# NethermindEth/cairo_zstd

Measured on AMD Instinct MI355X. Metric: decompressed MB/s (whole node), 128 KiB-block batch, higher is better.
Workload: dtype u8

## Files before the change

### cairo_zstd_amd/csrc/czstd_chain.hip

```cpp
#include "czstd_dict.h"

#ifndef CZC_SLOTS
#define CZC_SLOTS 10
#endif
#define CZC_LPS 4
static_assert(CZC_SLOTS * CZC_LPS <= 64, "quads of one wave");
#define CZC_MAXSYM 64
#define CZC_RING 512u
#define CZC_STEPS 32u
static_assert(((CZC_STEPS * 58u + 7u) / 8u + 12u) + 12u <= 256u + 12u, "a top-up adds at most 256 bytes: one must be enough for the next group");
#define CZC_NEED ((CZC_STEPS * 58u + 7u) / 8u + 12u)
#define CZC_MAP_WORDS CZ_CHAIN_MAP_WORDS

#define CZC_E16(nb, base, xb) ((uint16_t)(((((1u << (9u - (nb))) | ((base) >> (nb))) << 6) | (xb))))
#define CZC_E16_IDLE 0x8000u

struct CzChainSlot {
    uint16_t t_ll[512], t_ml[512], t_of[256];
    union {
        struct {
            __attribute__((aligned(16))) uint8_t stage[256];
            int16_t probs[3][CZC_MAXSYM];
            uint16_t counters_ml[CZC_MAXSYM];
        };
// ... 6 lines not shown
struct CzChainShared { CzChainSlot slot[CZC_SLOTS]; uint32_t llml[96]; uint16_t idle[2]; };

__device__ static inline __attribute__((always_inline)) int czc_fse_build_wave(uint16_t* table, const int16_t* probs, uint32_t nprobs, uint32_t log,
                                                                   uint8_t* symof, uint16_t* counters, const uint32_t* llml, uint32_t kind, cz_gptr map) {
    const uint32_t size = 1u << log, mask = size - 1, lim = kind == 0 ? 36u : (kind == 1 ? 32u : 53u);
    const uint32_t lane = (uint32_t)LANE;
    const unsigned long long lt = (1ull << lane) - 1ull;
    const int32_t p = lane < nprobs ? (int32_t)probs[lane] : 0;
    if (__ballot(p != 0 && lane >= lim)) return 1;
    const unsigned long long lowm = __ballot(p == -1);
    const uint32_t neg = size - (uint32_t)__popcll(lowm);
    if (p == -1) table[size - 1u - (uint32_t)__popcll(lowm & lt)] = (uint16_t)lane;
    counters[lane] = 0;
    const uint32_t cnt = p > 0 ? (uint32_t)p : 0u;
    const uint32_t cum = cz_wave_incl_scan(cnt) - cnt;
    for (uint32_t i = 4u * lane; i < size; i += 256u) *(uint32_t*)(symof + i) = 0u;
    cz_wave_sync();
    if (cnt && cum < size) symof[cum] = (uint8_t)lane;
    cz_wave_sync();
    {
        const uint32_t per = size >= 64u ? size >> 6 : 1u, b0 = lane * per;
        const int act = b0 < size;
        uint32_t run = 0, vals[8];
#pragma unroll
        for (uint32_t j = 0; j < 8; j++) { if (act && j < per) { const uint32_t v = symof[b0 + j]; run = v > run ? v : run; } vals[j] = run; }
        uint32_t inc = act ? run : 0u;
#define CZC_MAX_STEP(CTRL, RM) do { const uint32_t o_ = cz_dpp<CTRL, RM>(0u, inc); inc = o_ > inc ? o_ : inc; } while (0)
        CZC_MAX_STEP(CZ_DPP_SHR1, 0xF); CZC_MAX_STEP(CZ_DPP_SHR2, 0xF); CZC_MAX_STEP(CZ_DPP_SHR4, 0xF); CZC_MAX_STEP(CZ_DPP_SHR8, 0xF);
        CZC_MAX_STEP(CZ_DPP_BCAST15, 0xA); CZC_MAX_STEP(CZ_DPP_BCAST31, 0xC);
#undef CZC_MAX_STEP
        const uint32_t exc = cz_dpp<CZ_DPP_WAVE_SHR1, 0xF>(0u, inc);
#pragma unroll
        for (uint32_t j = 0; j < 8; j++) if (act && j < per) symof[b0 + j] = (uint8_t)(vals[j] > exc ? vals[j] : exc);
    }
    cz_wave_sync();
    {
        const uint32_t step = (size >> 1) + (size >> 3) + 3u;
        uint32_t running = 0;
        for (uint32_t j0 = 0; j0 < size; j0 += 64u) {
            const uint32_t j = j0 + lane, pos = (j * step) & mask;
            const int valid = j < size && pos < neg;
            const unsigned long long vm = __ballot(valid);
            if (valid) table[pos] = symof[running + (uint32_t)__popcll(vm & lt)];
            running += (uint32_t)__popcll(vm);
        }
    }
    cz_wave_sync();
    for (uint32_t i0 = 0; i0 < size; i0 += 64u) {
        const uint32_t i = i0 + lane;
        const int in = i < size, cell = in && i < neg;
        const uint32_t s = in ? (uint32_t)table[i] : 0u;
        unsigned long long same = __ballot(cell);
#pragma unroll
        for (uint32_t b = 0; b < 6; b++) { const int bit = (int)((s >> b) & 1u); const unsigned long long m = __ballot(bit); same &= bit ? m : ~m; }
        const uint32_t n = cell ? (uint32_t)probs[s] : 1u;
        const uint32_t k = (cell ? (uint32_t)counters[s] : 0u) + (uint32_t)__popcll(same & lt);
        cz_wave_sync();
        if (cell && (same >> lane) == 1ull) counters[s] = (uint16_t)(k + 1u);
        const uint32_t xb = kind == 1 ? s : (llml[(kind == 2 ? 40u : 0u) + s] >> 24);
        uint32_t nb = log, bl = 0;
        if (cell) {
            const uint32_t m = 1u << (cz_hbs(n) - 1), slices = (m == n) ? n : m * 2;
            const uint32_t dbl = slices - n, single = n - dbl, width = size >> (cz_hbs(slices) - 1);
            nb = cz_hbs(width) - 1;
            if (k < dbl) { bl = single * width + k * width * 2; nb += 1; }
            else bl = (k - dbl) * width;
        }
        if (in) { table[i] = CZC_E16(nb, bl, xb); if (map) map[i] = (uint8_t)s; }
        cz_wave_sync();
    }
    return 0;
}

__device__ static inline uint4 czc_load16(uintptr_t a, uintptr_t S, uintptr_t E) {
    uint4 v;
    if (a >= S && a + 16 <= E) { __builtin_memcpy(&v, (CZ_GLOBAL const void*)a, 16); return v; }
    if (a + 16 <= S || a >= E) { v.x = v.y = v.z = v.w = 0; return v; }
    uint32_t w[4] = {0, 0, 0, 0};
    for (uint32_t b = 0; b < 16; b++) { const uintptr_t q = a + b; if (q >= S && q < E) w[b >> 2] |= (uint32_t)(*(cz_gcptr)q) << (8 * (b & 3)); }
    v.x = w[0]; v.y = w[1]; v.z = w[2]; v.w = w[3];
    return v;
}
#define CZC_PF (16 / CZC_LPS)
struct CzcPre { uint4 v[CZC_PF]; };
__device__ static inline void czc_prefetch(CzcPre& pre, int has_slot, intptr_t lo, uintptr_t Sk, uintptr_t Ek) {
    const uint32_t j = (uint32_t)LANE & 3u;
#pragma unroll
    for (uint32_t r = 0; r < CZC_PF; r++) {
        const uint32_t c = j + r * CZC_LPS;
        if (has_slot) pre.v[r] = czc_load16((uintptr_t)lo - 16u * (c + 1), Sk, Ek);
    }
}
__device__ static inline void czc_commit(CzChainSlot& sk, int has_slot, intptr_t old_lo, intptr_t new_lo, const CzcPre& pre) {
    const uint32_t j = (uint32_t)LANE & 3u;
    const uint32_t cnt = has_slot ? (uint32_t)(old_lo - new_lo) >> 4 : 0u;
#pragma unroll
    for (uint32_t r = 0; r < CZC_PF; r++) {
        const uint32_t c = j + r * CZC_LPS;
        if (c < cnt) {
            const uint32_t slot = (uint32_t)(((uintptr_t)old_lo - 16u * (c + 1)) & (CZC_RING - 1));
            *(uint4*)&sk.ring[slot] = pre.v[r];
            if (slot == CZC_RING - 16) { *(uint32_t*)&sk.mirror[4] = pre.v[r].y; *(uint32_t*)&sk.mirror[8] = pre.v[r].z; *(uint32_t*)&sk.mirror[12] = pre.v[r].w; }
        }
    }
}
__device__ static inline uint64_t czc_window(const CzChainSlot& sl, int32_t u) {
    const uint32_t ba = ((uint32_t)u >> 3) & (CZC_RING - 4), ph = (uint32_t)u & 31;
    const uint32_t w2 = *(const uint32_t*)(sl.ring + ba), w1 = *(const uint32_t*)(sl.ring + ba - 4), w0 = *(const uint32_t*)(sl.ring + ba - 8);
    const uint64_t hi = (((uint64_t)w2 << 32) | w1), lo = (((uint64_t)w1 << 32) | w0);
    const uint32_t h = ph ? (uint32_t)(hi >> ph) : w1, l = ph ? (uint32_t)(lo >> ph) : w0;
    return ((uint64_t)h << 32) | l;
}

struct CzcLane {
    uint32_t E;
    uint32_t S;
    int32_t  u;
    uint32_t ph;
    uint32_t w0, w1, w2;
    uint32_t slow;
};
struct CzcRole {
    const uint16_t* tb;
    const uint8_t* ringm8;
    uint32_t m1, m2;
    uint32_t sh;
    uint32_t lane0;
    uint32_t sbits;
};
#define CZC_QP(a, b, c, d) ((a) | ((b) << 2) | ((c) << 4) | ((d) << 6))
template <int CTRL> __device__ static inline uint32_t czc_qp(uint32_t v) { return (uint32_t)__builtin_amdgcn_update_dpp(0, (int)v, CTRL, 0xF, 0xF, true); }

__device__ static inline void czc_ring_words(CzcLane& c, const CzcRole& ro) {
    const uint8_t* ba = ro.ringm8 + (__builtin_amdgcn_ubfe((uint32_t)c.u, 5, 7) << 2);
    c.w0 = *(const uint32_t*)ba; c.w1 = *(const uint32_t*)(ba + 4); c.w2 = *(const uint32_t*)(ba + 8);
    c.ph = (uint32_t)c.u & 31u;
}
__device__ static inline uint32_t czc_bits32(const CzcRole& ro, uint32_t v) {
    const uint8_t* ba = ro.ringm8 + (__builtin_amdgcn_ubfe(v, 5, 7) << 2);
    return __builtin_amdgcn_alignbit(*(const uint32_t*)(ba + 8), *(const uint32_t*)(ba + 4), v & 31u);
}
#define CZC_WIDE_STEPS 16u
static_assert((CZC_WIDE_STEPS * 89u + 7u) / 8u + 12u <= CZC_NEED && CZC_STEPS % CZC_WIDE_STEPS == 0, "a redone asm group is whole wide groups, each within the staged bytes");
__device__ static inline void czc_step(CzcLane& c, const CzcRole& ro, CZ_GLOBAL uint64_t* rec, int act, int last, int store) {
    const uint32_t n = (uint32_t)__builtin_clz(c.E);
    const uint32_t x = __builtin_amdgcn_ubfe(c.E, 16, 5);
    const uint32_t p = (n << 8) + x;
    const uint32_t T = p + czc_qp<CZC_QP(1, 2, 0, 3)>(p) + czc_qp<CZC_QP(2, 0, 1, 3)>(p);
    const uint32_t t1 = czc_qp<CZC_QP(0, 0, 0, 0)>(p) & ro.m1, t2 = czc_qp<CZC_QP(1, 1, 1, 1)>(p) & ro.m2;
    const uint32_t incl = (t1 + t2 + p) >> 8;
    const uint32_t a_ = T & 0xFFu;
    const uint32_t xh = czc_bits32(ro, (uint32_t)c.u - a_);
    const uint32_t bits = __builtin_amdgcn_ubfe(xh, (0u - incl) & 31u, n);
    const uint32_t window = czc_bits32(ro, (uint32_t)c.u);
    const uint32_t cS = c.S << ro.sh;
    const uint32_t H = cS + czc_qp<CZC_QP(1, 2, 0, 3)>(cS) + czc_qp<CZC_QP(2, 0, 1, 3)>(cS);
    if (act) {
        if (store) *rec = a_ <= 32 ? ((uint64_t)window | ((uint64_t)H << 32))
                                   : ((uint64_t)((uint32_t)c.u - ro.sbits) | ((uint64_t)(H | CZC_REC_WIDE) << 32));
        if (last) c.u -= (int32_t)a_;
        else {
            c.S = (((c.E >> 22) << n) | bits) & 511u;
            c.E = (uint32_t)ro.tb[c.S] << 16;
            c.u -= (int32_t)(a_ + (T >> 8));
        }
        czc_ring_words(c, ro);
    }
}

#if defined(__HIP_DEVICE_COMPILE__)
#define CZC_ASM_HEAD(WIN) \
    CZC_ASM_LGKM_E                                  \
    "v_ffbh_u32 v100, %[E]\n" \
    "v_and_or_b32 v101, %[E], %[XM], %[K64]\n" \
    "v_sub_u32 v102, v101, v100\n" \
    "v_lshrrev_b32 v103, 22, %[E]\n" \
    "v_and_b32 %[PH], 31, %[U]\n"                  \
    "v_add_u32_dpp v105, v102, v102 quad_perm:[1,2,0,3] row_mask:0xf bank_mask:0xf\n" \
    "v_and_b32_dpp v106, v102, %[M1] quad_perm:[0,0,0,0] row_mask:0xf bank_mask:0xf\n" \
    "v_and_b32_dpp v107, v102, %[M2] quad_perm:[1,1,1,1] row_mask:0xf bank_mask:0xf\n" \
    "v_add_u32_dpp v105, v102, v105 quad_perm:[2,0,1,3] row_mask:0xf bank_mask:0xf\n" \
    "v_add3_u32 v109, v106, v107, v102\n" \
    "s_waitcnt lgkmcnt(0)\n" \
    "v_sub_co_u32_sdwa v110, vcc, %[PH], v105 dst_sel:DWORD dst_unused:UNUSED_PAD src0_sel:DWORD src1_sel:BYTE_2\n"    \
    "v_alignbit_b32 " WIN ", %[W2], v125, %[PH]\n" \
// ... 125 lines not shown

#define CZC_ASMW_HEAD(WIN) \
    "s_waitcnt lgkmcnt(2)\n" \
    "v_ffbh_u32 v100, %[E]\n" \
    "v_and_or_b32 v101, %[E], %[XM], %[K64]\n" \
    "v_sub_u32 v102, v101, v100\n" \
    "v_lshrrev_b32 v103, 22, %[E]\n" \
    "v_sub_u32 v119, %[U], %[SB]\n"                \
    "v_add_u32_dpp v105, v102, v102 quad_perm:[1,2,0,3] row_mask:0xf bank_mask:0xf\n" \
    "v_and_b32_dpp v106, v102, %[M1] quad_perm:[0,0,0,0] row_mask:0xf bank_mask:0xf\n" \
    "v_and_b32_dpp v107, v102, %[M2] quad_perm:[1,1,1,1] row_mask:0xf bank_mask:0xf\n" \
    "v_add_u32_dpp v105, v102, v105 quad_perm:[2,0,1,3] row_mask:0xf bank_mask:0xf\n" \
    "v_add3_u32 v109, v106, v107, v102\n" \
    "v_bfe_u32 v108, v105, 16, 8\n" \
    "s_waitcnt lgkmcnt(0)\n" \
    "v_cmp_ge_u32 vcc, %[PH], v108\n" \
    "v_sub_u32 v110, %[PH], v108\n" \
    "v_alignbit_b32 " WIN ", v127, v126, %[PH]\n" \
    "v_cndmask_b32 v111, v126, v127, vcc\n" \
    "v_cndmask_b32 v112, v125, v126, vcc\n" \
    "v_cmp_gt_i32 vcc, %[N32], v110\n"             \
    "v_cmp_lt_u32_e64 s[12:13], 32, v108\n" \
    "s_nop 0\n" \
    "v_cndmask_b32 v111, v111, v125, vcc\n" \
    "v_cndmask_b32 v112, v112, v124, vcc\n" \
    "v_alignbit_b32 v113, v111, v112, v110\n" \
    "v_bfe_u32 v116, v113, v109, v100\n" \
    "v_lshl_or_b32 %[S], v103, v100, v116\n" \
    "v_lshl_add_u32 v117, %[S], 1, %[TB]\n" \
    "ds_read_u16_d16_hi %[E], v117\n"
#define CZC_ASMW_TAIL(STORE, WIN, H, NEXTH) \
    "v_cndmask_b32_e64 " WIN ", " WIN ", v119, s[12:13]\n" \
    "v_cndmask_b32_e64 v128, 0, %[FL], s[12:13]\n" \
    "v_or_b32 " H ", " H ", v128\n" \
    STORE \
    "v_lshl_add_u32 v118, %[S], %[SH], %[NK]\n" \
    "v_dot4c_i32_i8_e32 %[U], 0x01ff0001, v105\n" \
    "v_and_b32 v129, 31, v108\n" \
    "v_add_u32_dpp " NEXTH ", v118, v118 quad_perm:[1,2,0,3] row_mask:0xf bank_mask:0xf\n" \
    "v_add_u32_dpp " NEXTH ", v118, " NEXTH " quad_perm:[2,0,1,3] row_mask:0xf bank_mask:0xf\n" \
    "v_bfe_u32 v114, %[U], 5, 7\n" \
    "v_and_b32 %[PH], 31, %[U]\n" \
    "v_lshl_add_u32 v115, v114, 2, %[RB]\n" \
    "ds_read2_b32 v[124:125], v115 offset1:1\n" \
    "ds_read2_b32 v[126:127], v115 offset0:2 offset1:3\n"
#define CZC_ASMW_EVEN(OFF) CZC_ASMW_HEAD("v120") CZC_ASMW_TAIL("", "v120", "v121", "v123")
#define CZC_ASMW_ODD(OFF) CZC_ASMW_HEAD("v122") CZC_ASMW_TAIL(CZC_ASM_STORE(OFF), "v122", "v123", "v121")
#define CZC_ASMW_PAIR(A) CZC_ASMW_EVEN(A) CZC_ASMW_ODD(A)
__device__ static inline void czc_group_asm_wide(CzcLane& c, const CzcRole& ro, CZ_GLOBAL uint64_t* rec) {
    const uint32_t tb32 = (uint32_t)(uintptr_t)(__attribute__((address_space(3))) const uint16_t*)ro.tb;
    const uint32_t rb32 = (uint32_t)(uintptr_t)(__attribute__((address_space(3))) const uint8_t*)ro.ringm8 - 4u;
    const uint32_t tbm = tb32 - 1024u, nk = 0u - (512u << ro.sh), k64 = ro.lane0 ? 0x40000040u : 0x40u;
    c.S += 512u;
    asm volatile(
        "v_bfe_u32 v114, %[U], 5, 7\n"
        "v_lshl_add_u32 v115, v114, 2, %[RB]\n"
        "ds_read2_b32 v[124:125], v115 offset1:1\n"
        "ds_read2_b32 v[126:127], v115 offset0:2 offset1:3\n"
        "v_lshl_add_u32 v118, %[S], %[SH], %[NK]\n"
        "s_nop 1\n"
        "v_add_u32_dpp v121, v118, v118 quad_perm:[1,2,0,3] row_mask:0xf bank_mask:0xf\n"
        "v_add_u32_dpp v121, v118, v121 quad_perm:[2,0,1,3] row_mask:0xf bank_mask:0xf\n"
        CZC_ASMW_PAIR(0) CZC_ASMW_PAIR(16) CZC_ASMW_PAIR(32) CZC_ASMW_PAIR(48) CZC_ASMW_PAIR(64) CZC_ASMW_PAIR(80) CZC_ASMW_PAIR(96) CZC_ASMW_PAIR(112)
        CZC_ASMW_PAIR(128) CZC_ASMW_PAIR(144) CZC_ASMW_PAIR(160) CZC_ASMW_PAIR(176) CZC_ASMW_PAIR(192) CZC_ASMW_PAIR(208) CZC_ASMW_PAIR(224) CZC_ASMW_PAIR(240)
        "s_waitcnt lgkmcnt(0)\n"
        : [E] "+v"(c.E), [S] "+v"(c.S), [U] "+v"(c.u), [PH] "+v"(c.ph)
        : [TB] "v"(tbm), [RB] "v"(rb32), [M1] "v"(ro.m1 ? 0xFFu : 0u), [M2] "v"(ro.m2 ? 0xFFu : 0u), [SH] "v"(ro.sh), [NK] "v"(nk), [K64] "v"(k64),
          [SB] "v"(ro.sbits), [FL] "v"(CZC_REC_WIDE), [XM] "s"(0x1F0000u), [N32] "s"(-32), [RP] "v"(rec)
        : "memory", "vcc", "s12", "s13",
          "v100", "v101", "v102", "v103", "v105", "v106", "v107", "v108", "v109", "v110", "v111", "v112", "v113", "v114", "v115",
          "v116", "v117", "v118", "v119", "v120", "v121", "v122", "v123", "v124", "v125", "v126", "v127", "v128", "v129");
    c.S -= 512u;
    czc_ring_words(c, ro);
}
#endif

#ifdef CZ_PROFILE
#define CZC_PROF_ACC(i) do { const unsigned long long n_ = __builtin_amdgcn_s_memtime(); cprof[i] += n_ - ct_; ct_ = n_; } while (0)
#define CZC_PROF_CNT(i) do { cprof[i] += 1; } while (0)
#else
#define CZC_PROF_ACC(i) do { } while (0)
#define CZC_PROF_CNT(i) do { } while (0)
#endif
__device__ static inline uint32_t czc_q0(uint32_t v) { return (uint32_t)__shfl((int)v, LANE & ~3); }
__device__ static inline uint64_t czc_q0_64(uint64_t v) { return ((uint64_t)czc_q0((uint32_t)(v >> 32)) << 32) | czc_q0((uint32_t)v); }

struct CzsBlk { uint32_t type, blk_off, bsize;
                uint32_t lt, regen, lit_hdr, nseq, sbody, modes; };
struct CzsWalk { const uint8_t* src; uint64_t len, pos, end, h8; uint32_t h8sh, defined, has_checksum; int first, active, ok, have_tree; };
__device__ static inline uint64_t czs_ld8_issue(const uint8_t* src, uint64_t len, uint64_t at, uint32_t* sh) {
    const uint64_t a2 = at + 8 <= len ? at : len - 8;
    uint64_t v; __builtin_memcpy(&v, src + a2, 8);
    *sh = (uint32_t)(at - a2);
    return v;
}
__device__ static inline uint64_t czs_ld8_value(uint64_t raw, uint32_t sh) { return sh >= 8 ? 0 : raw >> (8 * sh); }
__device__ static inline uint64_t czs_ld8(const uint8_t* src, uint64_t len, uint64_t at) { uint32_t sh; const uint64_t v = czs_ld8_issue(src, len, at, &sh); return czs_ld8_value(v, sh); }
__device__ static inline void czs_begin(CzsWalk& w, const uint8_t* src, uint64_t len, int valid) {
    w.src = src; w.len = len; w.pos = 0; w.end = 0; w.h8 = 0; w.h8sh = 8; w.defined = 0; w.has_checksum = 0; w.first = 1; w.active = 0; w.ok = 0; w.have_tree = 0;
    if (!valid || len < 8 || len >= 0xFFFFFFF0ull) return;
    const uint64_t h0 = czs_ld8(src, len, 0);
    const uint32_t magic = (uint32_t)h0;
    const uint32_t d = (uint32_t)(h0 >> 32) & 0xFF;
    const uint32_t single = (d >> 5) & 1, didf = d & 3, dl = didf == 3 ? 4 : didf, flag = d >> 6;
    const uint32_t fl = flag == 0 ? (single ? 1u : 0u) : flag == 1 ? 2u : flag == 2 ? 4u : 8u;
    const uint32_t hl = 5 + (single ? 0 : 1) + dl + fl;
    if (magic != 0xFD2FB528u || len < hl) return;
    if (!single) { const uint32_t wd = (uint32_t)(h0 >> 40) & 0xFF; const uint64_t base = 1ull << (10 + (wd >> 3)); if (base + (base / 8) * (wd & 7) >= 4123168604160ull) return; }
    w.pos = hl; w.active = 1; w.has_checksum = (d >> 2) & 1; w.h8 = czs_ld8_issue(src, len, hl, &w.h8sh);
}
__device__ static inline void czs_dict_check(CzsWalk& w, const cz_dict_entry* dicts, uint32_t ndicts) {
    if (!w.active) return;
    const uint64_t h0 = czs_ld8(w.src, w.len, 0);
    const uint32_t d = (uint32_t)(h0 >> 32) & 0xFF, didf = d & 3, dl = didf == 3 ? 4 : didf, at = 5 + (((d >> 5) & 1) ? 0 : 1);
    uint32_t id = (uint32_t)(h0 >> (8 * at));
    if (at + dl > 8) id |= (uint32_t)(czs_ld8(w.src, w.len, 8) << (8 * (8 - at)));
    id = dl == 0 ? 0u : (dl == 4 ? id : id & ((1u << (8 * dl)) - 1u));
    if (cz_dict_find(dicts, ndicts, id) == CZ_DICT_UNKNOWN) { w.active = 0; w.ok = 0; }
}
__device__ static inline int czs_next(CzsWalk& w, uint32_t chain_min_nseq, CzsBlk& b) {
    const uint8_t* src = w.src; const uint64_t len = w.len;
    if (!w.active) return 0;
    do {
        uint64_t pos = w.pos;
        if (pos == ~0ull) { w.active = 0; w.ok = 1; return 0; }
        if (len - pos < 3) break;
        const uint64_t h = czs_ld8_value(w.h8, w.h8sh);
        const uint32_t b0 = (uint32_t)h & 0xFF, b1 = (uint32_t)(h >> 8) & 0xFF, b2 = (uint32_t)(h >> 16) & 0xFF;
        const uint32_t type = (b0 >> 1) & 3, size = (b0 >> 3) | (b1 << 5) | (b2 << 13), blast = b0 & 1;
        if (type == 3 || size > 128u * 1024u) break;
        const uint64_t body = pos + 3; const uint32_t content = type == 1 ? 1u : size;
        if (len - body < content) break;
        w.pos = blast ? ~0ull : body + content;
        if (blast) w.end = body + content;
        else w.h8 = czs_ld8_issue(src, len, body + content, &w.h8sh);
        b.type = type; b.blk_off = (uint32_t)body; b.bsize = size; b.lt = 0; b.regen = 0; b.lit_hdr = 0; b.nseq = 0; b.sbody = 0; b.modes = 0;
        if (type != 2) return 1;
        if (size == 0) break;
        const uint32_t l0 = (uint32_t)(h >> 24) & 0xFF, lt = l0 & 3, fmt = (l0 >> 2) & 3;
        const uint32_t need = lt <= 1 ? ((fmt == 0 || fmt == 2) ? 1u : (fmt == 1 ? 2u : 3u)) : (fmt <= 1 ? 3u : (fmt == 2 ? 4u : 5u));
        if (size < need) break;
        const uint32_t l1 = need > 1 ? (uint32_t)(h >> 32) & 0xFF : 0, l2 = need > 2 ? (uint32_t)(h >> 40) & 0xFF : 0, l3 = need > 3 ? (uint32_t)(h >> 48) & 0xFF : 0, l4 = need > 4 ? (uint32_t)(h >> 56) & 0xFF : 0;
        uint32_t upper, regen;
        if (lt <= 1) { regen = (fmt == 0 || fmt == 2) ? l0 >> 3 : (fmt == 1 ? (l0 >> 4) + (l1 << 4) : (l0 >> 4) + (l1 << 4) + (l2 << 12)); upper = lt == 1 ? 1u : regen; }
        else {
            regen = fmt <= 1 ? (l0 >> 4) + ((l1 & 0x3f) << 4) : (fmt == 2 ? (l0 >> 4) + (l1 << 4) + ((l2 & 3) << 12) : (l0 >> 4) + (l1 << 4) + ((l2 & 0x3f) << 12));
            upper = fmt <= 1 ? (l1 >> 6) + (l2 << 2) : (fmt == 2 ? (l2 >> 2) + (l3 << 6) : (l2 >> 6) + (l3 << 2) + (l4 << 10));
        }
        if (size - need < upper) break;
        if (lt == 3 && !w.have_tree) break;
        if (lt == 2) w.have_tree = 1;
        const uint32_t so = need + upper, sl_ = size - so;
        if (sl_ == 0) break;
        const uint64_t sq = czs_ld8(src, len, body + so);
        const uint32_t s0 = (uint32_t)sq & 0xFF, s1 = (uint32_t)(sq >> 8) & 0xFF, s2 = (uint32_t)(sq >> 16) & 0xFF;
        uint32_t n = 0, hb = 0;
        if (s0 == 0) { }
        else if (s0 <= 127) { if (sl_ < 2) break; n = s0; hb = 1; }
        else if (s0 <= 254) { if (sl_ < 3) break; n = ((s0 - 128) << 8) + s1; hb = 2; }
        else { if (sl_ < 4) break; n = s1 + (s2 << 8) + 0x7F00u; hb = 3; }
        b.lt = lt; b.regen = regen; b.lit_hdr = need;
        if (!n) return 1;
        if (w.first && n < chain_min_nseq) break;
        b.nseq = n; b.modes = (uint32_t)(sq >> (8 * hb)) & 0xFF; b.sbody = so + hb + 1;
        int undefined = 0;
        for (int t = 0; t < 3; t++) {
// ... 199 lines not shown
            early = good && !(pre & CZ_PRE_DONE) && first_hdr != 0 && !has_large && !big && a.exec_counter != nullptr;
            a.lit_first[f] = good ? (first_node ? first_node : 1) : 0; a.frame_pre[f] = pre | (wx ? CZ_PRE_WXLIST : 0u) | (big ? CZ_PRE_WXBIG : 0u) | (early ? CZ_PRE_EARLY : 0u);
        }
    }
    { const unsigned long long em = __ballot(early); if (em && LANE == __ffsll((long long)em) - 1) atomicAdd(&a.scan_ctl[211], (uint32_t)__popcll(em)); }
    if (a.wx_list) {
        const unsigned long long wm = __ballot(wx);
        if (wm) {
            uint32_t base = 0;
            if (LANE == __ffsll((long long)wm) - 1) base = atomicAdd(&a.scan_ctl[206], (uint32_t)__popcll(wm));
            base = (uint32_t)__shfl((int)base, __ffsll((long long)wm) - 1);
            if (wx) a.wx_list[base + (uint32_t)__popcll(wm & ((1ull << LANE) - 1ull))] = f;
        }
    }
    if (with_lits) {
        const unsigned long long todo = __ballot(valid && !(a.frame_pre[f < a.n ? f : 0] & CZ_PRE_DONE));
        if (LANE == 0 && todo) atomicAdd(&a.scan_ctl[204], (uint32_t)__popcll(todo));
    }
}

__device__ static inline __attribute__((always_inline)) int czc_parse_tables(cz_gcptr blk, uint32_t bsize, uint32_t sbody, uint32_t modes, uint32_t want, const uint8_t* stage, uint32_t stage_n,
                                       int16_t (*probs)[CZC_MAXSYM], uint32_t* info, int32_t* rle, uint32_t* bitoff) {
    uint32_t off = sbody;
    for (int t = 0; t < 3; t++) {
        const uint32_t md = (modes >> (6 - 2 * t)) & 3, max_log = t == 1 ? 8u : 9u;
        const int take = (want >> t) & 1u;
        if (md == 0) {
            if (take) {
                const int8_t* d = t == 0 ? CZ_LL_DEFAULT : t == 1 ? CZ_OF_DEFAULT : CZ_ML_DEFAULT;
                const uint32_t n = t == 0 ? 36u : t == 1 ? 29u : 53u, lg = t == 1 ? 5u : 6u;
                for (uint32_t s = 0; s < n; s++) probs[t][s] = d[s];
                *info = (*info & ~(0x3FFu << (10 * t))) | (((n - 1) | (lg << 6)) << (10 * t));
                rle[t] = -1;
            }
        } else if (md == 1) {
            if (off >= bsize) return 1;
            const uint32_t sym = blk[off]; off += 1;
            if (take) {
                if (sym >= (t == 0 ? 36u : (t == 1 ? 32u : 53u))) return 1;
                rle[t] = (int32_t)sym; *info &= ~(0x3FFu << (10 * t));
            }
        } else if (md == 2) {
            CzFBits br; br.g = (cz_gcptr)(blk + off); br.len = bsize - off; br.idx = 0; br.stage = stage; br.stage_lo = 0; br.stage_hi = 0;
            if (stage && off - sbody < stage_n) { br.stage = stage + (off - sbody); br.stage_hi = stage_n - (off - sbody); }
            uint32_t np, lg, used;
            const int into = take ? t : (want & 2u ? 1 : 2);
            if (cz_fse_read_probs_inl(br, max_log, probs[into], &np, &lg, &used, 100, CZC_MAXSYM) || np > CZC_MAXSYM || np == 0) return 1;
            if (take) { *info = (*info & ~(0x3FFu << (10 * t))) | (((np - 1) | (lg << 6)) << (10 * t)); rle[t] = -1; }
            off += used;
            if (off > bsize) return 1;
        }
        if ((want >> (t + 1)) == 0) break;
    }
    *bitoff = off;
    return 0;
}

#define CZC_SYNC() cz_wave_sync()
extern "C" __global__ void __launch_bounds__(CZ_WG_THREADS, 1) cz_chain_kernel(cz_batch_args a) {
    __shared__ CzChainShared cs;
    __builtin_amdgcn_s_setprio(3);
    for (uint32_t i = (uint32_t)LANE; i < 36; i += 64) cs.llml[i] = CZ_LL_BASE[i] | ((uint32_t)CZ_LL_BITS[i] << 24);
    for (uint32_t i = (uint32_t)LANE; i < 53; i += 64) cs.llml[40 + i] = CZ_ML_BASE[i] | ((uint32_t)CZ_ML_BITS[i] << 24);
    if (LANE < 2) cs.idle[LANE] = (uint16_t)CZC_E16_IDLE;
    __syncthreads();
    const uint32_t qk = (uint32_t)LANE >> 2, ql = (uint32_t)LANE & 3u;
    const int has_slot = qk < CZC_SLOTS;
    const int owner = has_slot && ql == 0;
    CzChainSlot& sl = cs.slot[has_slot ? qk : 0];
    CzcRole ro;
    ro.ringm8 = sl.ring - 8; ro.tb = cs.idle; ro.sbits = 0;
    ro.m1 = (ql == 1 || ql == 2) ? 0xFF00u : 0u; ro.m2 = ql == 2 ? 0xFF00u : 0u; ro.sh = ql == 3 ? 0u : 9u * ql; ro.lane0 = ql == 0;
    const uint16_t* my_table = ql == 0 ? sl.t_ll : (ql == 1 ? sl.t_ml : sl.t_of);
#ifdef CZ_PROFILE
    unsigned long long cprof[16] = {0, 0, 0, 0, 0, 0, 0, 0, 0, 0, 0, 0, 0, 0, 0, 0}, ct_ = __builtin_amdgcn_s_memtime();
#endif
    uint32_t ndesc = 0, nlarge = 0; for (int c = 0; c < 20; c++) { ndesc += a.scan_ctl[c]; if ((uint32_t)c >= CZ_BIG_BLOCK_CLASS) nlarge += a.scan_ctl[c]; }
    if (ndesc > a.blk_capacity) ndesc = a.blk_capacity;
    if (nlarge > ndesc) nlarge = ndesc;
    const uint32_t list_lo = a.chain_part == 2u ? nlarge : 0u, list_hi = a.chain_part == 1u ? nlarge : ndesc;
    uint32_t* const list_counter = a.chain_part == 2u ? &a.scan_ctl[212] : &a.scan_ctl[64];
    const int publish = a.chain_part == 1u;
    if (list_lo >= list_hi) { if (LANE == 0) atomicAdd(&a.scan_ctl[205], 1u); return; }
    int chain_live = 0, wide = 0, exhausted = 0;
    uint32_t qnseq = 0, done = 0, sbits = 0;
    uintptr_t S = 0, E = 0; intptr_t ring_base = 0, loaded_lo = 0;
    CZ_GLOBAL uint64_t* rec = nullptr;
    uint32_t o_frame = 0, o_nseq = 0, o_mapflags = 0, o_bitoff = 0, o_bad0 = 0; uint64_t o_hdr = 0; int o_have = 0, o_pub = 0;
    CzcLane c; c.E = (uint32_t)CZC_E16_IDLE << 16; c.S = 0; c.u = 0; c.ph = 0; c.w0 = c.w1 = c.w2 = 0; c.slow = 0;
    CzcPre pre;
    for (uint32_t r = 0; r < CZC_PF; r++) pre.v[r] = uint4{0, 0, 0, 0};
    for (;;) {
        if (__ballot(owner && !o_have && !exhausted)) {
            cz_gcptr blk = nullptr; uint32_t bsize = 0, sbody = 0, modes = 0; uint32_t def[3] = {0, 0, 0};
            int got = 0;
            if (owner && !o_have && !exhausted) {
                for (;;) {
                    const uint32_t idx = list_lo + atomicAdd(list_counter, 1u);
                    if (idx >= list_hi) { exhausted = 1; break; }
                    const cz_blk_desc d = a.blk_desc[idx];
                    if (!d.nseq) continue;
                    blk = (cz_gcptr)(a.in_base + a.in_off[d.frame] + d.blk_off); bsize = d.bsize; sbody = d.sbody; modes = d.modes;
                    def[0] = d.def[0]; def[1] = d.def[1]; def[2] = d.def[2];
                    o_frame = d.frame; o_nseq = d.nseq; o_hdr = d.hdr; o_have = 1; got = 1;
                    o_pub = publish && (a.frame_pre[d.frame] & CZ_PRE_WXBIG) != 0u;
                    break;
                }
            }
            {
                const uintptr_t base = (uintptr_t)blk + sbody;
                const uintptr_t bk = (uintptr_t)czc_q0_64((uint64_t)base), Sk = (uintptr_t)czc_q0_64((uint64_t)(uintptr_t)blk), Ek = Sk + czc_q0(bsize);
                CZC_SYNC();
                if (czc_q0((uint32_t)got) && has_slot) for (uint32_t cc = ql; cc < 16; cc += CZC_LPS) *(uint4*)&sl.stage[16 * cc] = czc_load16(bk + 16 * cc, Sk, Ek);
                CZC_SYNC();
            }
            CZC_PROF_ACC(8); CZC_PROF_CNT(13);
            uint32_t binfo = 0; int32_t rles[3] = {-1, -1, -1}; int bad = 0;
            if (got) {
                o_mapflags = 0;
                for (int t = 0; t < 3; t++) if (((modes >> (6 - 2 * t)) & 3) != 3) o_mapflags |= 1u << t;
                bad = czc_parse_tables(blk, bsize, sbody, modes, 7u, sl.stage, 256u, sl.probs, &binfo, rles, &o_bitoff);
            }
            CZC_PROF_ACC(9);
            for (int t = 0; t < 3; t++) {
                const int rep = got && !bad && ((modes >> (6 - 2 * t)) & 3) == 3;
                if (!__ballot(rep)) continue;
                cz_gcptr dblk = nullptr; uint32_t dbsize = 0, dsbody = 0, dmodes = 0;
                if (rep) {
                    if (def[t] >= ndesc) bad = 1;
                    else {
                        const cz_blk_desc dd = a.blk_desc[def[t]];
                        if (dd.frame != o_frame) bad = 1;
                        else { dblk = (cz_gcptr)(a.in_base + a.in_off[dd.frame] + dd.blk_off); dbsize = dd.bsize; dsbody = dd.sbody; dmodes = dd.modes; }
                    }
                }
                const int go = rep && !bad;
                {
                    const uintptr_t base = (uintptr_t)dblk + dsbody;
                    const uintptr_t bk = (uintptr_t)czc_q0_64((uint64_t)base), Sk = (uintptr_t)czc_q0_64((uint64_t)(uintptr_t)dblk), Ek = Sk + czc_q0(dbsize);
                    CZC_SYNC();
                    if (czc_q0((uint32_t)go) && has_slot) for (uint32_t cc = ql; cc < 16; cc += CZC_LPS) *(uint4*)&sl.stage[16 * cc] = czc_load16(bk + 16 * cc, Sk, Ek);
                    CZC_SYNC();
                }
                if (go) { uint32_t dummy; bad = czc_parse_tables(dblk, dbsize, dsbody, dmodes, 1u << t, sl.stage, 256u, sl.probs, &binfo, rles, &dummy); }
            }
            if (got && bad) { got = 0; o_have = 0; a.frame_first[o_frame] = 0; if (o_pub) CZ_ST_AGENT(&a.chain_arena[o_hdr + 3], (uint64_t)2); }
            if (got && a.exec_counter) {
                const uint32_t info = (binfo >> 10) & 0x3FFu, lg = info >> 6, np = (info & 63u) + 1u, n6 = (o_nseq + 63u) >> 6;
                uint32_t nearc = 0, farc = 0;
                if (rles[1] >= 0) { nearc = rles[1] >= 2 && rles[1] <= 13 ? 256u : 0u; farc = rles[1] >= 14 ? 256u : 0u; }
                else if (lg) {
                    for (uint32_t sy = 2; sy < np; sy++) { const int32_t pr = sl.probs[1][sy]; const uint32_t cnt = pr > 0 ? (uint32_t)pr : (pr < 0 ? 1u : 0u); if (sy <= 13u) nearc += cnt; else farc += cnt; }
                    nearc = (nearc << 8) >> lg; farc = (farc << 8) >> lg;
                }
                if (nearc) atomicAdd(a.chain_top + 5, (unsigned long long)nearc * n6);
                if (farc) atomicAdd(a.chain_top + 6, (unsigned long long)farc * n6);
                uint32_t longc = 0;
                for (int t = 0; t < 3; t += 2) {
                    const uint32_t inf = (binfo >> (10 * t)) & 0x3FFu, lgt = inf >> 6, npt = (inf & 63u) + 1u, lim = t == 0 ? 8u : 13u;
                    if (rles[t] >= 0) longc += (uint32_t)rles[t] > lim ? 256u : 0u;
                    else if (lgt) {
                        uint32_t cl = 0;
                        for (uint32_t sy = lim + 1u; sy < npt; sy++) { const int32_t pr = sl.probs[t][sy]; cl += pr > 0 ? (uint32_t)pr : 0u; }
                        longc += (cl << 8) >> lgt;
                    }
                }
                if (longc) atomicAdd(a.chain_top + 7, (unsigned long long)longc * n6);
            }
            CZC_PROF_ACC(10);
            {
                CZC_SYNC();
                int tbad = 0;
                for (unsigned long long need = __ballot(owner && got); need; need &= need - 1) {
                    const int ol = cz_unii(__ffsll((long long)need) - 1);
                    const uint32_t binf = cz_readlane(binfo, ol), mf = cz_readlane(o_mapflags, ol);
                    const uint64_t hk = ((uint64_t)cz_readlane((uint32_t)(o_hdr >> 32), ol) << 32) | cz_readlane((uint32_t)o_hdr, ol);
                    CzChainSlot& bs = cs.slot[(uint32_t)ol >> 2];
                    cz_gptr maps = (cz_gptr)(a.chain_arena + hk + 4);
                    int sbad = 0;
#pragma unroll 1
                    for (uint32_t o = 0; o < 3; o++) {
                        const uint32_t bk = o == 0 ? 0u : (o == 1 ? 2u : 1u);
                        const uint32_t info = (binf >> (10 * bk)) & 0x3FFu;
                        if (!(info >> 6)) continue;
                        uint16_t* table = bk == 0 ? bs.t_ll : (bk == 1 ? bs.t_of : bs.t_ml);
                        uint8_t* symof = bk == 1 ? bs.stage : (uint8_t*)bs.t_of;
                        cz_gptr map = !((mf >> bk) & 1u) ? (cz_gptr)nullptr : (bk == 0 ? maps : (bk == 2 ? maps + 512 : maps + 1024));
                        sbad |= czc_fse_build_wave(table, bs.probs[bk], (info & 63u) + 1u, info >> 6, symof, bs.counters_ml, cs.llml, bk, map);
                        cz_wave_sync();
                    }
                    if (sbad && LANE == ol) tbad = 1;
                }
                CZC_SYNC();
                if (got && tbad) { got = 0; o_have = 0; a.frame_first[o_frame] = 0; if (o_pub) CZ_ST_AGENT(&a.chain_arena[o_hdr + 3], (uint64_t)2); }
                if (got) for (int t = 0; t < 3; t++) if (rles[t] >= 0) {
                    uint16_t* table = t == 0 ? sl.t_ll : (t == 1 ? sl.t_of : sl.t_ml);
                    table[0] = CZC_E16(0u, 0u, t == 1 ? (uint32_t)rles[t] : (cs.llml[(t == 2 ? 40u : 0u) + (uint32_t)rles[t]] >> 24));
                    if ((o_mapflags >> t) & 1u) ((cz_gptr)(a.chain_arena + o_hdr + 4))[t == 0 ? 0 : (t == 2 ? 512 : 1024)] = (uint8_t)rles[t];
                }
                CZC_SYNC();
            }
            CZC_PROF_ACC(11);
            const int qgot = (int)czc_q0((uint32_t)got) && has_slot;
            const uint32_t gn = czc_q0(o_nseq);
            const uintptr_t gblk = (uintptr_t)czc_q0_64((uint64_t)(uintptr_t)blk);
            const uint32_t gbitoff = czc_q0(o_bitoff), gbsize = czc_q0(bsize);
            if (qgot) {
                S = gblk + gbitoff; E = gblk + gbsize; qnseq = gn; done = 0; wide = 0;
                sbits = (uint32_t)(S & (CZC_RING - 1)) * 8u;
                ring_base = (intptr_t)(S & ~(uintptr_t)(CZC_RING - 1));
                const intptr_t hi = (intptr_t)((E + 15) & ~(uintptr_t)15);
                loaded_lo = hi - 256;
                czc_prefetch(pre, 1, hi, S, E);
                czc_commit(sl, 1, hi, loaded_lo, pre);
            }
            CZC_SYNC();
            if (qgot) czc_prefetch(pre, 1, loaded_lo, S, E);
            int32_t u0 = 0; uint32_t st_ll = 0, st_of = 0, st_ml = 0;
            if (got) {
                int32_t p = (int32_t)(E - S) * 8; int skipped = 0;
                o_bad0 = 0;
                for (;;) {
                    const uint32_t b = p > 0 ? (uint32_t)(czc_window(sl, (int32_t)sbits + p) >> 63) : 0; p -= 1; skipped++;
                    if (b == 1 || skipped > 8) break;
                }
                if (skipped > 8) o_bad0 = 1;
                uint32_t stv[3] = {0, 0, 0};
                for (int t = 0; t < 3; t++) {
                    if (rles[t] >= 0) continue;
                    const uint32_t lg = (binfo >> (10 * t + 6)) & 15u;
                    stv[t] = p > 0 ? (uint32_t)(czc_window(sl, (int32_t)sbits + p) >> (64 - lg)) : 0; p -= (int32_t)lg;
                }
                st_ll = stv[0]; st_of = stv[1]; st_ml = stv[2];
                if (p < 0) o_bad0 = 1;
                u0 = (int32_t)sbits + p;
            }
            {
                const uint32_t qll = czc_q0(st_ll), qml = czc_q0(st_ml), qof = czc_q0(st_of), qu = czc_q0((uint32_t)u0);
                const uint64_t qh = czc_q0_64(o_hdr);
                if (qgot) {
                    c.u = (int32_t)qu; c.slow = 0; ro.sbits = sbits;
                    c.S = ql == 0 ? qll : (ql == 1 ? qml : (ql == 2 ? qof : 0u));
                    if (ql == 3) { ro.tb = cs.idle; c.S = 0; } else ro.tb = my_table;
                    c.E = (uint32_t)ro.tb[c.S] << 16;
                    czc_ring_words(c, ro);
                    rec = (CZ_GLOBAL uint64_t*)(a.chain_arena + qh + 4 + CZC_MAP_WORDS);
                    chain_live = 1;
                }
            }
            CZC_PROF_ACC(1);
        }
        if (!__ballot(chain_live)) { if (!__ballot(owner && !exhausted)) break; continue; }
        {
            const int32_t uq = (int32_t)czc_qp<CZC_QP(0, 0, 0, 0)>((uint32_t)c.u);
            const intptr_t curb = ring_base + ((uq > 0 ? uq - 1 : 0) >> 3);
            const int need = chain_live && (curb - (intptr_t)CZC_NEED < loaded_lo);
            if (__ballot(need)) {
                intptr_t new_lo = chain_live ? ((curb - (intptr_t)(CZC_RING - 4) + 15) & ~(intptr_t)15) : loaded_lo;
                if (new_lo > loaded_lo) new_lo = loaded_lo;
                if (new_lo < loaded_lo - 256) new_lo = loaded_lo - 256;
                CZC_SYNC();
                czc_commit(sl, chain_live, loaded_lo, new_lo, pre);
                loaded_lo = new_lo;
                CZC_SYNC();
                czc_prefetch(pre, chain_live, loaded_lo, S, E);
                if (chain_live) czc_ring_words(c, ro);
                CZC_PROF_ACC(2); CZC_PROF_CNT(5);
            }
        }
        {
            const uint32_t left = qnseq - done;
            const int tail = __ballot(chain_live && left <= CZC_STEPS) != 0;
            int ran_asm = 0;
            (void)tail; (void)wide;
#if defined(__HIP_DEVICE_COMPILE__)
            if (!tail && !(a.debug_flags & CZ_DEBUG_CHAIN_CPP_STEP)) {
                CZ_GLOBAL uint64_t* rp = chain_live && ql < 3 ? rec + done : (CZ_GLOBAL uint64_t*)(a.chain_arena + 8);
                if (!__ballot(chain_live && wide)) {
                    const CzcLane sv = c;
                    c.slow = 0;
#ifdef CZC_EXP_OLD_STEP
                    czc_group_asm(c, ro, rp);
#else
                    czc_group_asm2(c, ro, rp);
#endif
                    const int hit = chain_live && ql < 3 && c.slow > 32;
                    if (__ballot(hit)) { wide |= (int)czc_q0((uint32_t)hit); c = sv; }
                }
                if (__ballot(chain_live && wide)) czc_group_asm_wide(c, ro, rp);
                if (chain_live) done += CZC_STEPS;
                ran_asm = 1;
            }
#endif
            if (!ran_asm) {
                const uint32_t steps = !chain_live ? 0u : (left < CZC_WIDE_STEPS ? left : CZC_WIDE_STEPS);
                for (uint32_t i = 0; i < CZC_WIDE_STEPS; i++) czc_step(c, ro, rec + done + i, i < steps, done + i + 1 == qnseq, ql == 0);
                done += steps;
            }
            CZC_PROF_ACC(3); CZC_PROF_CNT(6);
        }
        if (__ballot(chain_live && done >= qnseq)) {
            const int fin = chain_live && done >= qnseq;
            int fbad = 0;
            if (fin && owner) {
                fbad = o_bad0 || c.u - (int32_t)sbits != 0;
                if (fbad) a.frame_first[o_frame] = 0;
                else { uint64_t* h = a.chain_arena + o_hdr; h[0] = ((uint64_t)o_nseq << 32) | o_mapflags; h[1] = o_bitoff; if (!o_pub) h[3] = 0; }
                o_have = 0;
            }
            if (__ballot(fin && owner && o_pub)) {
                CZ_RELEASE_AGENT();
                if (fin && owner && o_pub) CZ_ST_AGENT(&a.chain_arena[o_hdr + 3], (uint64_t)(fbad ? 2 : 1));
            }
            if (fin) { chain_live = 0; wide = 0; ro.tb = cs.idle; c.S = 0; c.E = (uint32_t)CZC_E16_IDLE << 16; }
            CZC_PROF_ACC(4);
        }
    }
#ifdef CZ_PROFILE
    if (LANE == 0 && a.prof) { for (int i = 0; i < 8; i++) atomicAdd(&a.prof[32 + i], cprof[i]); for (int i = 8; i < 14; i++) atomicAdd(&a.prof[50 + i - 8], cprof[i]); }
#endif
    if (LANE == 0) atomicAdd(&a.scan_ctl[205], 1u);
}
```

Before: 179,600.

## Hold chain ring prefetch in AGPRs with partial vmcnt waits and simplify ballots

```diff
diff --git a/cairo_zstd_amd/csrc/czstd_chain.hip b/cairo_zstd_amd/csrc/czstd_chain.hip
--- a/cairo_zstd_amd/csrc/czstd_chain.hip
+++ b/cairo_zstd_amd/csrc/czstd_chain.hip
@@ -112,25 +112,73 @@
     return v;
 }
 #define CZC_PF (16 / CZC_LPS)
+#ifdef CZC_EXP_NOSTORE
+#define CZC_GROUP_STORES 0u
+#else
+#define CZC_GROUP_STORES (CZC_STEPS / 2u)
+#endif
+#if defined(__HIP_DEVICE_COMPILE__)
+struct CzcPre { };
+#define CZC_PRE_PIECE(A0, A1, A2, A3, has, adr) do { \
+        if (has) { \
+            if ((adr) >= Sk && (adr) + 16 <= Ek) \
+                asm volatile("global_load_dwordx4 a[" #A0 ":" #A3 "], %0, off" :: "v"((CZ_GLOBAL const void*)(adr)) : "memory", "a" #A0, "a" #A1, "a" #A2, "a" #A3); \
+            else if ((adr) + 16 <= Sk || (adr) >= Ek)    \
+                asm volatile("v_accvgpr_write_b32 a" #A0 ", 0\nv_accvgpr_write_b32 a" #A1 ", 0\nv_accvgpr_write_b32 a" #A2 ", 0\nv_accvgpr_write_b32 a" #A3 ", 0" \
+                             ::: "memory", "a" #A0, "a" #A1, "a" #A2, "a" #A3); \
+            else {                                       \
+                const uint4 v_ = czc_load16(adr, Sk, Ek); \
+                asm volatile("v_accvgpr_write_b32 a" #A0 ", %0\nv_accvgpr_write_b32 a" #A1 ", %1\nv_accvgpr_write_b32 a" #A2 ", %2\nv_accvgpr_write_b32 a" #A3 ", %3" \
+                             :: "v"(v_.x), "v"(v_.y), "v"(v_.z), "v"(v_.w) : "memory", "a" #A0, "a" #A1, "a" #A2, "a" #A3); \
+            } \
+        } \
+    } while (0)
+__device__ static inline void czc_pre_settle() { asm volatile("s_waitcnt vmcnt(0)" ::: "memory"); }
+__device__ static inline void czc_prefetch(CzcPre&, int has_slot, intptr_t lo, uintptr_t Sk, uintptr_t Ek) {
+    const uintptr_t a0 = (uintptr_t)lo - 16u * (((uint32_t)LANE & 3u) + 1);
+    static_assert(CZC_PF == 4 && CZC_LPS == 4, "a[0:15], pieces 64 bytes apart");
+    CZC_PRE_PIECE(0, 1, 2, 3, has_slot, a0);
+    CZC_PRE_PIECE(4, 5, 6, 7, has_slot, a0 - 64);
+    CZC_PRE_PIECE(8, 9, 10, 11, has_slot, a0 - 128);
+    CZC_PRE_PIECE(12, 13, 14, 15, has_slot, a0 - 192);
+}
+__device__ static inline void czc_pre_take(const CzcPre&, uint32_t since, uint4* v) {
+    if (since >= 48u) asm volatile("s_waitcnt vmcnt(48)" ::: "memory");
+    else if (since >= 32u) asm volatile("s_waitcnt vmcnt(32)" ::: "memory");
+    else if (since >= 16u) asm volatile("s_waitcnt vmcnt(16)" ::: "memory");
+    else asm volatile("s_waitcnt vmcnt(0)" ::: "memory");
+    asm volatile("v_accvgpr_read_b32 %0, a0\nv_accvgpr_read_b32 %1, a1\nv_accvgpr_read_b32 %2, a2\nv_accvgpr_read_b32 %3, a3\n"
+                 "v_accvgpr_read_b32 %4, a4\nv_accvgpr_read_b32 %5, a5\nv_accvgpr_read_b32 %6, a6\nv_accvgpr_read_b32 %7, a7\n"
+                 "v_accvgpr_read_b32 %8, a8\nv_accvgpr_read_b32 %9, a9\nv_accvgpr_read_b32 %10, a10\nv_accvgpr_read_b32 %11, a11\n"
+                 "v_accvgpr_read_b32 %12, a12\nv_accvgpr_read_b32 %13, a13\nv_accvgpr_read_b32 %14, a14\nv_accvgpr_read_b32 %15, a15"
+                 : "=v"(v[0].x), "=v"(v[0].y), "=v"(v[0].z), "=v"(v[0].w), "=v"(v[1].x), "=v"(v[1].y), "=v"(v[1].z), "=v"(v[1].w),
+                   "=v"(v[2].x), "=v"(v[2].y), "=v"(v[2].z), "=v"(v[2].w), "=v"(v[3].x), "=v"(v[3].y), "=v"(v[3].z), "=v"(v[3].w)
+                 :: "memory");
+}
+#else
 struct CzcPre { uint4 v[CZC_PF]; };
 __device__ static inline void czc_prefetch(CzcPre& pre, int has_slot, intptr_t lo, uintptr_t Sk, uintptr_t Ek) {
     const uint32_t j = (uint32_t)LANE & 3u;
-#pragma unroll
     for (uint32_t r = 0; r < CZC_PF; r++) {
         const uint32_t c = j + r * CZC_LPS;
         if (has_slot) pre.v[r] = czc_load16((uintptr_t)lo - 16u * (c + 1), Sk, Ek);
     }
 }
-__device__ static inline void czc_commit(CzChainSlot& sk, int has_slot, intptr_t old_lo, intptr_t new_lo, const CzcPre& pre) {
+__device__ static inline void czc_pre_settle() { }
+__device__ static inline void czc_pre_take(const CzcPre& pre, uint32_t, uint4* v) { for (uint32_t r = 0; r < CZC_PF; r++) v[r] = pre.v[r]; }
+#endif
+__device__ static inline void czc_commit(CzChainSlot& sk, int has_slot, int32_t old_lo, int32_t new_lo, const CzcPre& pre, uint32_t since) {
     const uint32_t j = (uint32_t)LANE & 3u;
     const uint32_t cnt = has_slot ? (uint32_t)(old_lo - new_lo) >> 4 : 0u;
+    uint4 v[CZC_PF];
+    czc_pre_take(pre, since, v);
 #pragma unroll
     for (uint32_t r = 0; r < CZC_PF; r++) {
         const uint32_t c = j + r * CZC_LPS;
         if (c < cnt) {
-            const uint32_t slot = (uint32_t)(((uintptr_t)old_lo - 16u * (c + 1)) & (CZC_RING - 1));
-            *(uint4*)&sk.ring[slot] = pre.v[r];
-            if (slot == CZC_RING - 16) { *(uint32_t*)&sk.mirror[4] = pre.v[r].y; *(uint32_t*)&sk.mirror[8] = pre.v[r].z; *(uint32_t*)&sk.mirror[12] = pre.v[r].w; }
+            const uint32_t slot = ((uint32_t)old_lo - 16u * (c + 1)) & (CZC_RING - 1);
+            *(uint4*)&sk.ring[slot] = v[r];
+            if (slot == CZC_RING - 16) { *(uint32_t*)&sk.mirror[4] = v[r].y; *(uint32_t*)&sk.mirror[8] = v[r].z; *(uint32_t*)&sk.mirror[12] = v[r].w; }
         }
     }
 }
@@ -422,6 +470,13 @@
 #define CZC_PROF_ACC(i) do { } while (0)
 #define CZC_PROF_CNT(i) do { } while (0)
 #endif
+#define CZC_LO_DEAD (-(1 << 30))
+#define CZC_NSEQ_DEAD 0xFFFFFFFFu
+#if defined(__HIP_DEVICE_COMPILE__)
+__device__ static inline bool czc_any(bool b) { return __builtin_amdgcn_ballot_w64(b) != 0; }
+#else
+__device__ static inline bool czc_any(bool b) { return __ballot(b ? 1 : 0) != 0; }
+#endif
 __device__ static inline uint32_t czc_q0(uint32_t v) { return (uint32_t)__shfl((int)v, LANE & ~3); }
 __device__ static inline uint64_t czc_q0_64(uint64_t v) { return ((uint64_t)czc_q0((uint32_t)(v >> 32)) << 32) | czc_q0((uint32_t)v); }
 
@@ -787,16 +842,20 @@
     uint32_t* const list_counter = a.chain_part == 2u ? &a.scan_ctl[212] : &a.scan_ctl[64];
     const int publish = a.chain_part == 1u;
     if (list_lo >= list_hi) { if (LANE == 0) atomicAdd(&a.scan_ctl[205], 1u); return; }
-    int chain_live = 0, wide = 0, exhausted = 0;
-    uint32_t qnseq = 0, done = 0, sbits = 0;
-    uintptr_t S = 0, E = 0; intptr_t ring_base = 0, loaded_lo = 0;
+    int chain_live = 0, wide = 0, exhausted = owner ? 0 : 1;
+    uint32_t qnseq = CZC_NSEQ_DEAD, done = 0, sbits = 0;
+    uintptr_t S = 0, E = 0; intptr_t ring_base = 0;
+    int32_t lo_rel = CZC_LO_DEAD;
     CZ_GLOBAL uint64_t* rec = nullptr;
+    CZ_GLOBAL uint64_t* const sink = (CZ_GLOBAL uint64_t*)(a.chain_arena + 8);
+    CZ_GLOBAL uint64_t* rp = sink; uint32_t rp_step = 0;
+    (void)rp;
     uint32_t o_frame = 0, o_nseq = 0, o_mapflags = 0, o_bitoff = 0, o_bad0 = 0; uint64_t o_hdr = 0; int o_have = 0, o_pub = 0;
     CzcLane c; c.E = (uint32_t)CZC_E16_IDLE << 16; c.S = 0; c.u = 0; c.ph = 0; c.w0 = c.w1 = c.w2 = 0; c.slow = 0;
-    CzcPre pre;
-    for (uint32_t r = 0; r < CZC_PF; r++) pre.v[r] = uint4{0, 0, 0, 0};
+    CzcPre pre = {};
+    uint32_t since = 0;
     for (;;) {
-        if (__ballot(owner && !o_have && !exhausted)) {
+        if (czc_any((o_have | exhausted) == 0)) {
             cz_gcptr blk = nullptr; uint32_t bsize = 0, sbody = 0, modes = 0; uint32_t def[3] = {0, 0, 0};
             int got = 0;
             if (owner && !o_have && !exhausted) {
@@ -914,13 +973,14 @@
                 S = gblk + gbitoff; E = gblk + gbsize; qnseq = gn; done = 0; wide = 0;
                 sbits = (uint32_t)(S & (CZC_RING - 1)) * 8u;
                 ring_base = (intptr_t)(S & ~(uintptr_t)(CZC_RING - 1));
-                const intptr_t hi = (intptr_t)((E + 15) & ~(uintptr_t)15);
-                loaded_lo = hi - 256;
-                czc_prefetch(pre, 1, hi, S, E);
-                czc_commit(sl, 1, hi, loaded_lo, pre);
-            }
+                lo_rel = (int32_t)((intptr_t)((E + 15) & ~(uintptr_t)15) - ring_base) - 256;
+            }
+            czc_pre_settle();
+            czc_prefetch(pre, qgot, ring_base + lo_rel + 256, S, E);
+            czc_commit(sl, qgot, lo_rel + 256, lo_rel, pre, 0u);
             CZC_SYNC();
-            if (qgot) czc_prefetch(pre, 1, loaded_lo, S, E);
+            czc_prefetch(pre, qgot, ring_base + lo_rel, S, E);
+            since = 0;
             int32_t u0 = 0; uint32_t st_ll = 0, st_of = 0, st_ml = 0;
             if (got) {
                 int32_t p = (int32_t)(E - S) * 8; int skipped = 0;
@@ -950,50 +1010,57 @@
                     c.E = (uint32_t)ro.tb[c.S] << 16;
                     czc_ring_words(c, ro);
                     rec = (CZ_GLOBAL uint64_t*)(a.chain_arena + qh + 4 + CZC_MAP_WORDS);
+                    if (ql < 3) { rp = rec; rp_step = CZC_STEPS; }
                     chain_live = 1;
                 }
             }
             CZC_PROF_ACC(1);
         }
-        if (!__ballot(chain_live)) { if (!__ballot(owner && !exhausted)) break; continue; }
+        if (!czc_any(chain_live != 0)) { if (!czc_any(exhausted == 0)) break; continue; }
         {
             const int32_t uq = (int32_t)czc_qp<CZC_QP(0, 0, 0, 0)>((uint32_t)c.u);
-            const intptr_t curb = ring_base + ((uq > 0 ? uq - 1 : 0) >> 3);
-            const int need = chain_live && (curb - (intptr_t)CZC_NEED < loaded_lo);
-            if (__ballot(need)) {
-                intptr_t new_lo = chain_live ? ((curb - (intptr_t)(CZC_RING - 4) + 15) & ~(intptr_t)15) : loaded_lo;
-                if (new_lo > loaded_lo) new_lo = loaded_lo;
-                if (new_lo < loaded_lo - 256) new_lo = loaded_lo - 256;
+            const int32_t cur = ((uq > 0 ? uq : 1) - 1) >> 3;
+            if (czc_any(cur - (int32_t)CZC_NEED < lo_rel)) {
+                int32_t new_lo = chain_live ? ((cur - (int32_t)(CZC_RING - 4) + 15) & ~15) : lo_rel;
+                if (new_lo > lo_rel) new_lo = lo_rel;
+                if (new_lo < lo_rel - 256) new_lo = lo_rel - 256;
                 CZC_SYNC();
-                czc_commit(sl, chain_live, loaded_lo, new_lo, pre);
-                loaded_lo = new_lo;
+                czc_commit(sl, chain_live, lo_rel, new_lo, pre, since);
+                lo_rel = new_lo;
                 CZC_SYNC();
-                czc_prefetch(pre, chain_live, loaded_lo, S, E);
+                czc_prefetch(pre, chain_live, ring_base + lo_rel, S, E);
+                since = 0;
                 if (chain_live) czc_ring_words(c, ro);
                 CZC_PROF_ACC(2); CZC_PROF_CNT(5);
             }
         }
         {
             const uint32_t left = qnseq - done;
-            const int tail = __ballot(chain_live && left <= CZC_STEPS) != 0;
+            const bool tail = czc_any(left <= CZC_STEPS);
             int ran_asm = 0;
             (void)tail; (void)wide;
 #if defined(__HIP_DEVICE_COMPILE__)
             if (!tail && !(a.debug_flags & CZ_DEBUG_CHAIN_CPP_STEP)) {
-                CZ_GLOBAL uint64_t* rp = chain_live && ql < 3 ? rec + done : (CZ_GLOBAL uint64_t*)(a.chain_arena + 8);
-                if (!__ballot(chain_live && wide)) {
-                    const CzcLane sv = c;
+                bool any_wide = czc_any(wide != 0);
+                if (!any_wide) {
+                    const uint32_t sv_E = c.E, sv_S = c.S; const int32_t sv_u = c.u;
                     c.slow = 0;
 #ifdef CZC_EXP_OLD_STEP
                     czc_group_asm(c, ro, rp);
 #else
                     czc_group_asm2(c, ro, rp);
 #endif
-                    const int hit = chain_live && ql < 3 && c.slow > 32;
-                    if (__ballot(hit)) { wide |= (int)czc_q0((uint32_t)hit); c = sv; }
-                }
-                if (__ballot(chain_live && wide)) czc_group_asm_wide(c, ro, rp);
+                    since += CZC_GROUP_STORES;
+                    if (czc_any(c.slow > 32)) {
+                        const int hit = chain_live && ql < 3 && c.slow > 32;
+                        wide |= (int)czc_q0((uint32_t)hit);
+                        c.E = sv_E; c.S = sv_S; c.u = sv_u; czc_ring_words(c, ro);
+                        any_wide = true;
+                    }
+                }
+                if (any_wide) { czc_group_asm_wide(c, ro, rp); since += CZC_GROUP_STORES; }
                 if (chain_live) done += CZC_STEPS;
+                rp += rp_step;
                 ran_asm = 1;
             }
 #endif
@@ -1001,10 +1068,11 @@
                 const uint32_t steps = !chain_live ? 0u : (left < CZC_WIDE_STEPS ? left : CZC_WIDE_STEPS);
                 for (uint32_t i = 0; i < CZC_WIDE_STEPS; i++) czc_step(c, ro, rec + done + i, i < steps, done + i + 1 == qnseq, ql == 0);
                 done += steps;
+                if (rp_step) rp += steps;
             }
             CZC_PROF_ACC(3); CZC_PROF_CNT(6);
         }
-        if (__ballot(chain_live && done >= qnseq)) {
+        if (czc_any(done >= qnseq)) {
             const int fin = chain_live && done >= qnseq;
             int fbad = 0;
             if (fin && owner) {
@@ -1017,7 +1085,7 @@
                 CZ_RELEASE_AGENT();
                 if (fin && owner && o_pub) CZ_ST_AGENT(&a.chain_arena[o_hdr + 3], (uint64_t)(fbad ? 2 : 1));
             }
-            if (fin) { chain_live = 0; wide = 0; ro.tb = cs.idle; c.S = 0; c.E = (uint32_t)CZC_E16_IDLE << 16; }
+            if (fin) { chain_live = 0; wide = 0; ro.tb = cs.idle; c.S = 0; c.E = (uint32_t)CZC_E16_IDLE << 16; rp = sink; rp_step = 0; qnseq = CZC_NSEQ_DEAD; done = 0; lo_rel = CZC_LO_DEAD; }
             CZC_PROF_ACC(4);
         }
     }
```

Result: faster. 183,300, median of 6 (+2.1%).
